# pedroand6/Voxel-Raytracer

Measured on AMD Instinct MI355X. Metric: Mrays/s at 1920×1080 primary rays; achieved HBM GB/s vs peak, higher is better.
Workload: dtype f32

## Files before the change

voxel-raytracer_amd/__init__.py:

```python
import ctypes as C
import os
import subprocess

import numpy as np

HERE = os.path.dirname(os.path.abspath(__file__))
CSRC = os.path.join(HERE, "csrc")
HIP_LIB = os.environ.get("VRT_HIP_LIB") or os.path.join(HERE, "libvrt_hip.so")
HOST_LIB = os.path.join(HERE, "libvrt_host.so")
TEST_LIB = os.path.join(HERE, "libvrt_hip_test.so")
OPT_RAY_TABLES, OPT_EMPTY_OCTANTS, OPT_DISPLAY_KERNEL, OPT_FULL_OPAQUE, OPT_HEAVY_TILES, OPT_MISS_TILES = 1, 2, 3, 4, 5, 6

MODE_PRIMARY, MODE_PRIMARY_SHADOW, MODE_FULL = 0, 1, 2
MODES = {"primary": MODE_PRIMARY, "primary_shadow": MODE_PRIMARY_SHADOW, "full": MODE_FULL}
ACCUM_JITTER = 1
TONEMAP_CLAMP, TONEMAP_REINHARD = 0, 1
TONEMAPS = {"clamp": TONEMAP_CLAMP, "reinhard": TONEMAP_REINHARD}


class Tonemap(C.Structure):
    _fields_ = [("op", C.c_int32), ("exposure", C.c_float)]


class VrtError(RuntimeError):
# ... 501 lines not shown
    cp = np.ascontiguousarray(cam_pos, np.float32)
    iv = np.ascontiguousarray(inv_view, np.float32)
    out = (C.c_int32 * 12)()
    r = L.vrt_test_lens_select(t.ctypes.data if t.size else None, t.size, (C.c_int32 * 3)(*world_min), (C.c_int32 * 3)(*world_max),
                               float(voxel_scale), _fptr(cp), _fptr(iv), float(aperture), out)
    if r != 0:
        raise VrtError(f"vrt_test_lens_select failed ({r})")
    return dict(box_valid=bool(out[0]), eye_shared=bool(out[1]), first_shared=bool(out[2]), no_medium=bool(out[3]),
                empty=bool(out[4]), lo=tuple(out[5:8]), hi=tuple(out[8:11]), root_shift=int(out[11]))


def miss_mask(texels, inv_proj, inv_view, cam_pos, width, height, voxel_scale=1.0, world_min=(-1023, -1023, -1023),
              world_max=(1024, 1024, 1024)):
    L = test_lib()
    L.vrt_test_miss_mask.argtypes = [C.c_void_p, C.c_size_t, C.POINTER(C.c_int32), C.POINTER(C.c_int32), C.c_float,
                                     C.POINTER(C.c_float), C.POINTER(C.c_float), C.POINTER(C.c_float), C.c_int, C.c_int,
                                     C.c_void_p, C.POINTER(C.c_int32)]
    t = np.ascontiguousarray(texels, np.uint8)
    ip = np.ascontiguousarray(inv_proj, np.float32).reshape(-1)
    iv = np.ascontiguousarray(inv_view, np.float32).reshape(-1)
    cp = np.zeros(4, np.float32)
    cp[:len(cam_pos)] = np.asarray(cam_pos, np.float32).reshape(-1)[:4]
    mask = np.zeros(((height + 7) // 8, (width + 7) // 8), np.uint8)
    stats = (C.c_int32 * 2)()
    r = L.vrt_test_miss_mask(t.ctypes.data if t.size else None, t.size, (C.c_int32 * 3)(*world_min), (C.c_int32 * 3)(*world_max),
                             float(voxel_scale), _fptr(ip), _fptr(iv), _fptr(cp), int(width), int(height), mask.ctypes.data, stats)
    if r < 0:
        raise VrtError(f"vrt_test_miss_mask failed ({r})")
    if r == 0:
        return None
    return mask, int(stats[0]), bool(stats[1])


def test_tile_order(tile_ticks, wave_slots, device=0):
    L = test_lib()
    t = np.ascontiguousarray(tile_ticks, np.uint32).reshape(-1)
    assert t.size % 4 == 0
    n = t.size // 4
    L.vrt_test_tile_order.argtypes = [C.c_int, C.c_void_p, C.c_uint32, C.c_uint32, C.c_void_p, C.c_void_p]
    order = np.zeros(n, np.uint32)
    split = np.zeros(1, np.uint32)
    r = L.vrt_test_tile_order(device, t.ctypes.data, n, wave_slots, order.ctypes.data, split.ctypes.data)
    if r:
        raise VrtError(f"vrt_test_tile_order failed ({r})")
    return order, int(split[0])



def tree_is_opaque(texels):
    L = test_lib()
    L.vrt_test_tree_is_opaque.argtypes = [C.c_void_p, C.c_size_t]
    t = np.ascontiguousarray(texels, np.uint8)
    r = L.vrt_test_tree_is_opaque(t.ctypes.data if t.size else None, t.size)
    if r < 0:
        raise VrtError(f"vrt_test_tree_is_opaque failed ({r})")
    return r == 1


def view_in_range(inv_view):
    m = np.ascontiguousarray(inv_view, np.float32).reshape(16)
    return test_lib().vrt_test_view_in_range(m.ctypes.data) == 1


def wide_find(texels, points, world_min=(-1023, -1023, -1023), world_max=(1024, 1024, 1024)):
    L = test_lib()
    t = np.ascontiguousarray(texels, np.uint8)
# ... 525 lines not shown
```

voxel-raytracer_amd/csrc/vrt_args.h:

```cpp
#pragma once
#include <hip/hip_runtime.h>
#include <stdint.h>

namespace vrt {

struct F3 { float x, y, z; };
struct I3 { int x, y, z; };

constexpr int kMaxViews = 4;
constexpr int kGroupTiles = 4;
constexpr int kSplitParts = 8, kSplitMaxGroups = 64;
struct View {
    float inv_proj[16];
    float inv_view[16];
    float cam_pos[4];
    uint32_t *out_rgba;
    int2 *out_id;
    uint32_t eye0, eye1;
    uint32_t first_w0, first_w1, first_node, first_anode;
    int first_s, first_as, first_valid;
    const float *gen_x, *gen_y;
    float gen_z;
    uint32_t gen_fast;
    const uint8_t *miss;
    uint32_t miss_stamp;
};

struct ViewSet {
    View v[kMaxViews];
};

struct KArgs {
    int n_views;
    float voxel_scale;
    int wmin[3];
    int wmax[3];
    float global_light[4];
    float light_dir[3];
    float light_inv[3], light_push[3], light_dposf[3];
    int light_dpos[3];
    int shade_fast;
    int highlighted[3];
    int tex_dim;
    int width, height;
    int row0, n_rows, tile_rows, row_stride;
    int compact;
    uint32_t tiles_x_magic;
    int row_mode;
    const uint2 *nodes;
    uint32_t n_records;
    uint32_t lds_records;
    const uint2 *cells;
    const uint2 *cells4;
    uint32_t n_roots;
    const uint32_t *root_table;
    uint32_t root0_node;
    int root0_shift;
// ... 15 lines not shown
```

voxel-raytracer_amd/csrc/vrt_common.hip.h:

```cpp
#pragma once

#include "vrt_args.h"

namespace vrt {

#define VRT_DEV __device__ __forceinline__

VRT_DEV float fmin_c(float a, float b) { return b < a ? b : a; }
VRT_DEV float fmax_c(float a, float b) { return a < b ? b : a; }
VRT_DEV float dot3(F3 a, F3 b) { return (a.x * b.x + a.y * b.y) + a.z * b.z; }
VRT_DEV float len3(F3 a) { return __builtin_sqrtf(dot3(a, a)); }
VRT_DEV F3 scale3(F3 a, float s) { return F3{a.x * s, a.y * s, a.z * s}; }
VRT_DEV F3 add3(F3 a, F3 b) { return F3{a.x + b.x, a.y + b.y, a.z + b.z}; }
VRT_DEV F3 sub3(F3 a, F3 b) { return F3{a.x - b.x, a.y - b.y, a.z - b.z}; }
VRT_DEV F3 normalize3(F3 a) { return scale3(a, 1.0f / __builtin_sqrtf(dot3(a, a))); }

VRT_DEV float rcp_inrange(float x) {
    float y = __builtin_amdgcn_rcpf(x);
    y = __builtin_fmaf(__builtin_fmaf(-x, y, 1.0f), y, y);
    const float q = __builtin_fmaf(__builtin_fmaf(-x, y, 1.0f), y, y);
    return __builtin_fmaf(__builtin_fmaf(-x, q, 1.0f), y, q);
}
VRT_DEV float sqrt_inrange(float x) {
    const float s = __builtin_amdgcn_sqrtf(x);
// ... 186 lines not shown
}

VRT_DEV void record_find(const KArgs &a, I3 p, uint32_t &w0, uint32_t &w1) {
    w0 = w1 = 0u;
    if (!in_world(a, p)) return;
    int mn[3] = {a.wmin[0], a.wmin[1], a.wmin[2]}, mx[3] = {a.wmax[0], a.wmax[1], a.wmax[2]};
    const int q[3] = {p.x, p.y, p.z};
    uint32_t rec = 0u;
    for (int i = 0; i < 16; ++i) {
        uint32_t ci = 0u;
#pragma unroll
        for (int k = 0; k < 3; ++k) {
            const int mid = mn[k] + ((mx[k] - mn[k]) >> 1);
            const bool hi = q[k] >= mid;
            if (hi) { ci |= 1u << (2 - k); mn[k] = mid; } else mx[k] = mid;
        }
        const uint2 r = a.nodes[rec];
        const uint32_t bit = 1u << ci;
        if (!(r.x & bit)) return;
        const uint32_t idx = r.y + (uint32_t)__builtin_popcount(r.x & 0xffu & (bit - 1u));
        if (idx >= a.n_records) return;
        if (r.x & (bit << 8)) { const uint2 l = a.nodes[idx]; w0 = l.x; w1 = l.y; return; }
        rec = idx;
    }
}

template <class T, class = void> struct host_light { static constexpr bool value = false; };
template <class T> struct host_light<T, decltype((void)T::kHostLight)> { static constexpr bool value = T::kHostLight; };
template <class T, class = void> struct miss_tiles { static constexpr bool value = false; };
template <class T> struct miss_tiles<T, decltype((void)T::kMissTiles)> { static constexpr bool value = T::kMissTiles; };

VRT_DEV bool miss_forward(F3 d) {
    return (d.x > 0.0f || d.x < -2e-8f) && (d.y > 0.0f || d.y < -2e-8f) && (d.z > 0.0f || d.z < -2e-8f);
}

constexpr uint32_t kSeedPlanes = 5, kSeedValid = 1u << 31;
struct Seed { F3 hp; uint32_t word; float iof; };

template <int MODE, class TRAV, bool JIT = false, bool LENS = false, bool MISS = false, bool HDR = false>
VRT_DEV void trace_pixel(const KArgs &a, const View &vw, const typename TRAV::Ctx &tc_, int px, int py, uint32_t &rgba, int2 &idd, LateOut &lo,
                         uint32_t *seed = nullptr, Seed *seed_regs = nullptr, uint32_t sample = 0u, const LensRay *lens = nullptr,
                         uint32_t miss_byte = 0u, float *fc_out = nullptr) {
    const float kPI = 3.14159265359f;
    const LensRay pr = pixel_ray<JIT, LENS>(a, vw, px, py, sample, lens);
    F3 ray_dir = pr.dir, ray_origin = pr.o;
    uint32_t eye0 = pr.eye0, eye1 = pr.eye1;

    int voxel_id = 0;
    int pixel_dist = a.wmax[0] - a.wmin[0];
    F3 gro = scale3(ray_origin, a.voxel_scale);
    Decoded tvd = decode_leaf(eye0, eye1);
    float start_iof = (tvd.p[0] > 0.0f && tvd.p[0] < 3.0f) ? tvd.p[0] : 1.0f;
    float medium_density = tvd.c[3] * 5.0f;
    float mc[3] = {1.0f, 1.0f, 1.0f};
    if (tvd.c[3] > 0.0f) { mc[0] = tvd.c[0]; mc[1] = tvd.c[1]; mc[2] = tvd.c[2]; }
    float fc[3] = {0.0f, 0.0f, 0.0f};
    const float sky[3] = {0.5f, 0.7f, 1.0f};

    Hit h;
    uint32_t seed_word = 0u;
    float seed_iof = 1.0f;
    const uint32_t eye_b = eye1 & 0xffu;
    const uint32_t iof_byte = (eye_b >= 1u && eye_b <= 254u) ? eye_b : 85u;
    bool hit = false;
    bool miss_tile = false;
    if constexpr (MISS) {
// ... 191 lines not shown
            uint32_t rgba;
            int2 idd;
            const View &vw = vs.v[blockIdx.y];
            LateOut lo;
            if constexpr (MODE == 5) {
                const uint32_t *sp = reinterpret_cast<const uint32_t *>(a.defer_rec) + ((size_t)tile * kSeedPlanes) * 64 + lane;
                Seed seed;
                seed.word = sp[3 * 64];
                seed.hp = F3{0.0f, 0.0f, 0.0f};
                seed.iof = 1.0f;
                if (seed.word & kSeedValid) {
                    seed.hp = F3{__uint_as_float(sp[0]), __uint_as_float(sp[64]), __uint_as_float(sp[2 * 64])};
                    seed.iof = __uint_as_float(sp[4 * 64]);
                }
                if (full::bounce_pixel<TRAV>(a, tc_, px, py, seed, rgba)) {
                    const LateArgs la = late_args();
                    const LateView lv_ = late_view();
                    lv_->out_rgba[(size_t)(la->compact ? j : py) * (size_t)la->width + (size_t)px] = rgba;
                }
            } else {
            if constexpr (MODE == 2)
                full::trace_pixel_full<TRAV>(a, vw, tc_, px, py, rgba, idd, lo);
            else if constexpr (MODE == 4)
                trace_pixel<1, TRAV>(a, vw, tc_, px, py, rgba, idd, lo, reinterpret_cast<uint32_t *>(a.defer_rec) + ((size_t)tile * kSeedPlanes) * 64 + lane);
            else if constexpr (MODE == 6) {
                Seed seed;
                seed.word = 0u;
                trace_pixel<1, TRAV>(a, vw, tc_, px, py, rgba, idd, lo, nullptr, &seed);
                uint32_t both;
                if (full::bounce_pixel<TRAV>(a, tc_, px, py, seed, both)) rgba = both;
            }
            else if constexpr ((MODE == 0 || MODE == 1) && miss_tiles<TRAV>::value) {
                uint32_t miss_byte = vw.miss_stamp;
                if (vw.miss) {
                    miss_byte = vw.miss[8u + (uint32_t)(py >> 3) * (uint32_t)((a.width + 7) >> 3) + (uint32_t)(px >> 3)];
                    if (*reinterpret_cast<const uint32_t *>(vw.miss) == vw.miss_stamp) miss_byte = vw.miss_stamp;
                }
                trace_pixel<MODE, TRAV, false, false, true>(a, vw, tc_, px, py, rgba, idd, lo, nullptr, nullptr, 0u, nullptr, miss_byte);
            }
            else trace_pixel<MODE, TRAV>(a, vw, tc_, px, py, rgba, idd, lo);
            if constexpr (MODE == 0) lo = LateOut{vw.out_rgba, vw.out_id, a.width, a.compact};
            size_t o = (size_t)(lo.compact ? j : py) * (size_t)lo.width + (size_t)px;
            if (lo.out_rgba) lo.out_rgba[o] = rgba;
            if (lo.out_id) lo.out_id[o] = idd;
            }
        }
        if constexpr (SCHED & 2) {
#ifndef VRT_EXP_STATS
            if (part_wave) { if (lane == 0) atomicMax(&a.tile_cost[tile], (uint32_t)(((__builtin_readcyclecounter() - t_begin) * 21ull) >> 4)); }
            else if (lane == 0) a.tile_cost[tile] = (uint32_t)(__builtin_readcyclecounter() - t_begin);
#endif
        }
    }
}

}
```

voxel-raytracer_amd/csrc/vrt_dispatch.cpp:

```cpp
#include "vrt_internal.h"

#include <algorithm>
#include <cmath>
#include <cstdio>
#include <new>

using namespace vrt_internal;
#include "vrt_launch.h"

namespace vrt_internal {

SchedState *sched_state(vrt_ctx *c, hipStream_t s, int width, int n_rows, int row0, int row_stride, int tile_rows, int mode,
                        uint32_t n_tiles, uint32_t n_groups) {
    uint64_t &tick = c->sched_tick;
    ++tick;
    for (SchedState &st : c->sched)
        if (st.stream == s && st.width == width && st.n_rows == n_rows && st.row0 == row0 && st.row_stride == row_stride &&
            st.tile_rows == tile_rows && st.mode == mode && st.n_tiles == n_tiles && st.n_groups == n_groups) {
            st.last_use = tick;
            return &st;
        }
    SchedState *slot = nullptr;
    if (c->sched.size() < kSchedMaxStates) {
        c->sched.emplace_back();
// ... 84 lines not shown
    if (hipMemcpy(t->d_tab, tab.data(), tab.size() * sizeof(float), hipMemcpyHostToDevice) != hipSuccess) return nullptr;
    t->fit_ok = miss_table_fit(tab.data(), z, W, H, t->fit);
    t->ok = true;
    return t;
}

bool occupancy(vrt_ctx *c) {
    vrt_ctx::Occupancy &o = c->occ;
    const bool same = o.built && o.tree_gen == c->tree_gen && std::memcmp(o.wmin, c->params.world_min, sizeof o.wmin) == 0 &&
                      std::memcmp(o.wmax, c->params.world_max, sizeof o.wmax) == 0;
    if (same) return o.ok;
    o.built = true; o.ok = false;
    o.tree_gen = c->tree_gen;
    std::memcpy(o.wmin, c->params.world_min, sizeof o.wmin);
    std::memcpy(o.wmax, c->params.world_max, sizeof o.wmax);
    for (int k = 0; k < 3; ++k)
        if (o.wmin[k] < -vrt::miss::kMaxWorld || o.wmax[k] > vrt::miss::kMaxWorld) return false;
    std::vector<int> boxes;
    if (!vrt::occupancy_boxes(c->host_records, o.wmin, o.wmax, (size_t)vrt::miss::kMaxBoxes, boxes)) return false;
    const size_t bytes = boxes.size() * sizeof(int);
    if (hipDeviceSynchronize() != hipSuccess) return false;
    if (bytes > o.capacity) {
        (void)hipFree(o.d_boxes);
        o.d_boxes = nullptr; o.capacity = 0;
        if (hipMalloc((void **)&o.d_boxes, bytes) != hipSuccess) { (void)hipGetLastError(); return false; }
        o.capacity = bytes;
    }
    if (bytes && hipMemcpy(o.d_boxes, boxes.data(), bytes, hipMemcpyHostToDevice) != hipSuccess) { (void)hipGetLastError(); return false; }
    o.n_boxes = boxes.size() / 6;
    o.ok = true;
    return true;
}

const uint8_t *miss_mask(vrt_ctx *c, const vrt::View &w, const vrt_ctx::RayTable &t, float voxel_scale, hipStream_t s, uint32_t &stamp) {
    vrt_ctx::Occupancy &o = c->occ;
    if (o.seen_gen != c->tree_gen || std::memcmp(o.seen_wmin, c->params.world_min, sizeof o.seen_wmin) != 0 ||
        std::memcmp(o.seen_wmax, c->params.world_max, sizeof o.seen_wmax) != 0) {
        o.seen_gen = c->tree_gen;
        std::memcpy(o.seen_wmin, c->params.world_min, sizeof o.seen_wmin);
        std::memcpy(o.seen_wmax, c->params.world_max, sizeof o.seen_wmax);
        o.stable = 0;
    }
    const uint64_t need = std::max<uint64_t>(vrt::miss::kStableMin, c->host_records.size() / vrt::miss::kStablePerRecords);
    if (o.stable < need) { ++o.stable; return nullptr; }
    const float gro[3] = {w.cam_pos[0] * voxel_scale, w.cam_pos[1] * voxel_scale, w.cam_pos[2] * voxel_scale};
    if (!vrt::miss::eye_in_world(gro, c->params.world_min, c->params.world_max)) return nullptr;
    const int W = t.width, H = t.height;
    vrt_ctx::MissMask *hit = nullptr, *lru = nullptr;
    for (auto &m : c->miss_masks) {
        if (m.width == W && m.height == H && m.tree_gen == c->tree_gen && std::memcmp(m.wmin, c->params.world_min, sizeof m.wmin) == 0 &&
            std::memcmp(m.wmax, c->params.world_max, sizeof m.wmax) == 0 && std::memcmp(m.inv_proj, w.inv_proj, sizeof m.inv_proj) == 0 &&
            std::memcmp(m.inv_view, w.inv_view, sizeof m.inv_view) == 0 && std::memcmp(m.gro, gro, sizeof m.gro) == 0)
            hit = &m;
        if (!lru || m.last_use < lru->last_use) lru = &m;
    }
    if (hit && !hit->pending) {
        hit->last_use = ++c->miss_tick;
        if (!hit->ok) return nullptr;
        if (hit->stream != s) {
            if (hipStreamWaitEvent(s, hit->built, 0) != hipSuccess) { (void)hipGetLastError(); return nullptr; }
            hit->shared = true;
        }
        stamp = hit->stamp;
        return reinterpret_cast<const uint8_t *>(hit->d_mask);
    }
    if (!hit) {
        vrt_ctx::MissMask *m;
        if (c->miss_masks.size() < 8) {
            c->miss_masks.emplace_back();
            m = &c->miss_masks.back();
        } else {
            m = lru;
        }
        std::memcpy(m->inv_proj, w.inv_proj, sizeof m->inv_proj);
        std::memcpy(m->inv_view, w.inv_view, sizeof m->inv_view);
        std::memcpy(m->gro, gro, sizeof m->gro);
        m->width = W; m->height = H; m->tree_gen = c->tree_gen;
        std::memcpy(m->wmin, c->params.world_min, sizeof m->wmin);
        std::memcpy(m->wmax, c->params.world_max, sizeof m->wmax);
        m->ok = false;
        m->pending = true;
        m->last_use = ++c->miss_tick;
        return nullptr;
    }
    vrt_ctx::MissMask *m = hit;
    m->pending = false;
    m->last_use = ++c->miss_tick;
    vrt::miss::ViewParams vp;
    if (!t.fit_ok || !miss_view_params(w.inv_view, gro, t.fit, vp)) return nullptr;
    if (!m->built && hipEventCreateWithFlags(&m->built, hipEventDisableTiming) != hipSuccess) { m->built = nullptr; (void)hipGetLastError(); return nullptr; }
    if (!occupancy(c)) return nullptr;
    if (m->d_mask && (m->shared || m->stream != s) && hipDeviceSynchronize() != hipSuccess) return nullptr;
    const size_t bytes = 8 + (size_t)vp.tiles_x * (size_t)vp.tiles_y;
    if (bytes > m->capacity) {
        if (m->d_mask && hipDeviceSynchronize() != hipSuccess) return nullptr;
        uint32_t *fresh = nullptr;
        if (hipMalloc((void **)&fresh, bytes) != hipSuccess) { (void)hipGetLastError(); return nullptr; }
        (void)hipFree(m->d_mask);
        m->d_mask = fresh;
        m->capacity = bytes;
        m->stamp = 0;
    }
    if (m->stamp == 255u) m->stamp = 0u;
    m->stamp = (uint8_t)(m->stamp + 1u);
    if (m->stamp == 1u && hipMemsetAsync(m->d_mask, 0, m->capacity, s) != hipSuccess) { (void)hipGetLastError(); return nullptr; }
    if (vrt::launch::miss_mask(vp, c->occ.d_boxes, (uint32_t)c->occ.n_boxes, m->d_mask, m->stamp, s) != hipSuccess ||
        hipEventRecord(m->built, s) != hipSuccess) {
        (void)hipGetLastError();
        return nullptr;
    }
    m->stream = s;
    m->shared = false;
    m->ok = true;
    stamp = m->stamp;
    return reinterpret_cast<const uint8_t *>(m->d_mask);
}

int enqueue(vrt_ctx *c, int width, int height, int row0, int n_rows, int tile_rows, int row_stride, int compact,
            int mode, void *d_rgba, void *d_id, hipStream_t s, const vrt_view *views, int n_views, const AccumStep *acc) {
    if (!c->have_scene) return vrt_fail(c, VRT_E_STATE, "vrt_dispatch: no octree uploaded (call vrt_upload_octree first)");
    if (c->batch.open) return vrt_fail(c, VRT_E_STATE, "vrt_dispatch: a patch batch is open (call vrt_patch_end first)");
    if (!views && !c->have_camera) return vrt_fail(c, VRT_E_STATE, "vrt_dispatch: no camera set (call vrt_set_camera first)");
    if (n_views < 1 || n_views > vrt::kMaxViews) return vrt_fail(c, VRT_E_INVALID, "vrt_dispatch_views: 1 to 4 views per launch");
    if (mode != VRT_MODE_PRIMARY && mode != VRT_MODE_PRIMARY_SHADOW && mode != VRT_MODE_FULL)
        return vrt_fail(c, VRT_E_INVALID, "unknown mode");
    if (n_rows <= 0) return VRT_OK;
    {
        const int ra = ensure_analysis(c);
        if (ra) return ra;
    }
    Variant v = *find_variant(c->variant);
    if (v.trav >= 3 && !c->wide_ok) { v.trav = 2; v.wpe = 1; }
    if (v.trav == 2 && c->unit_internal) v.trav = 1;
    if (mode == VRT_MODE_FULL) {
        if (v.trav >= 3) v.wpe = 5;
    } else if (!acc && mode == VRT_MODE_PRIMARY_SHADOW && c->variant == 20 && v.trav == 3) {
        v.wpe = 7;
    }
    vrt::KArgs a;
    vrt::ViewSet vs;
    std::memset(&vs, 0, sizeof vs);
    a.n_views = n_views;
    int eyes[vrt::kMaxViews][3];
    const vrt_ctx::RayTable *tables[vrt::kMaxViews] = {};
    for (int i = 0; i < n_views; ++i) {
        vrt::View &w = vs.v[i];
        std::memcpy(w.inv_proj, views ? views[i].inv_projection : c->inv_proj, sizeof w.inv_proj);
        std::memcpy(w.inv_view, views ? views[i].inv_view : c->inv_view, sizeof w.inv_view);
        std::memcpy(w.cam_pos, views ? views[i].camera_pos : c->cam_pos, sizeof w.cam_pos);
        w.out_rgba = (uint32_t *)(views ? views[i].d_rgba8 : d_rgba);
        w.out_id = (int2 *)(views ? views[i].d_id_dist : d_id);
        int eye[3];
        for (int k = 0; k < 3; ++k) {
            const float g = floorf(w.cam_pos[k] * c->params.voxel_scale);
            eye[k] = g != g ? 0 : (g >= 2147483648.0f ? 2147483647 : (g < -2147483648.0f ? (-2147483647 - 1) : (int)g));
        }
        for (int k = 0; k < 3; ++k) eyes[i][k] = eye[k];
        vrt::eye_lookup(c->host_records, c->params.world_min, c->params.world_max, eye, w.eye0, w.eye1);
        vrt::FirstFind ff;
        w.first_valid = (c->wide_ok && vrt::first_find(c->wide, c->params.world_min, c->params.world_max, eye, vrt::v3::kAnchorShift, ff)) ? 1 : 0;
        if (w.first_valid) {
            w.first_w0 = ff.w0; w.first_w1 = ff.w1; w.first_node = ff.node; w.first_anode = ff.anode;
            w.first_s = ff.s; w.first_as = ff.as;
        }
        w.gen_x = w.gen_y = nullptr; w.gen_z = 0.0f; w.gen_fast = 0u;
        w.miss = nullptr;
        w.miss_stamp = 0u;
        tables[i] = nullptr;
        if (view_matrix_in_range(w.inv_view)) {
            if (const vrt_ctx::RayTable *t = ray_table(c, w.inv_proj, width, height)) {
                w.gen_x = t->d_tab; w.gen_y = t->d_tab + width; w.gen_z = t->z; w.gen_fast = 1u;
                tables[i] = t;
            }
        }
    }
    const bool lens = acc && acc->aperture > 0.0f;
    vrt::LensSel lsel;
    if (lens) {
        vrt::lens_select(c->host_records, c->wide_ok ? &c->wide : nullptr, c->params.world_min, c->params.world_max,
                         c->params.voxel_scale, vs.v[0].cam_pos, vs.v[0].inv_view, acc->aperture, lsel);
        if (!lsel.first_shared) vs.v[0].first_valid = 0;
    }
    if (v.trav == 4 && mode != VRT_MODE_FULL) {
        bool eye_in_medium = false;
        for (int i = 0; i < n_views; ++i) {
            const uint32_t b = vs.v[i].eye1 & 0xffu;
            eye_in_medium = eye_in_medium || (b >= 1u && b <= 254u && b != 85u);
        }
        if (lens) eye_in_medium = !lsel.no_medium;
        if (eye_in_medium) { v.trav = 3; v.wpe = 6; }
    }
    if (c->miss_tiles_on && !acc && v.trav == 4 && v.wpe == 7 && mode != VRT_MODE_FULL)
        for (int i = 0; i < n_views; ++i)
            if (tables[i]) vs.v[i].miss = miss_mask(c, vs.v[i], *tables[i], c->params.voxel_scale, s, vs.v[i].miss_stamp);
    a.voxel_scale = c->params.voxel_scale;
    for (int i = 0; i < 3; ++i) {
        a.wmin[i] = c->params.world_min[i];
        a.wmax[i] = c->params.world_max[i];
        a.light_dir[i] = c->params.light_dir[i];
        a.highlighted[i] = c->params.highlighted[i];
        const float d = a.light_dir[i];
        a.light_inv[i] = (fabsf(d) < 1e-8f) ? 1e20f : 1.0f / d;
        a.light_push[i] = (d > 0.0f ? 1.0f : (d < 0.0f ? -1.0f : 0.0f)) * 0.001f;
        a.light_dpos[i] = d > 0.0f ? 1 : 0;
        a.light_dposf[i] = d > 0.0f ? 1.0f : 0.0f;
    }
    for (int i = 0; i < 4; ++i) a.global_light[i] = c->params.global_light[i];
    a.shade_fast = 1;
    for (int i = 0; i < 3; ++i)
        if (!(fabsf(a.global_light[i]) <= 1073741824.0f) || !(fabsf(a.light_dir[i]) <= 1073741824.0f)) a.shade_fast = 0;
    a.tex_dim = (int)c->info.tex_dim;
    a.width = width;
    a.height = height;
    a.row0 = row0;
    a.n_rows = n_rows;
    a.tile_rows = tile_rows;
    a.row_stride = row_stride;
    a.compact = compact;
    a.nodes = c->d_nodes;
    a.n_records = c->info.n_records;
    a.lds_records = 0u;
    a.cells = c->d_cells;
    a.cells4 = c->d_cells ? c->d_cells + c->cells_capacity : nullptr;
    a.n_roots = c->wide_ok ? (uint32_t)c->wide.roots.size() : 0u;
    for (int k = 0; k < 3; ++k) a.root0_min[k] = a.n_roots ? c->wide.roots[0].origin[k] : 0;
    a.root_table = c->d_roots;
    a.root0_node = a.n_roots ? c->wide.roots[0].node : 0u;
// ... 422 lines not shown
```

voxel-raytracer_amd/csrc/vrt_internal.h:

```cpp
#pragma once
#include "../../include/vrt.h"

#include <hip/hip_runtime.h>

#include <cstring>
#include <string>
#include <vector>

#include "vrt_args.h"
#include "vrt_layout.h"
#include "vrt_miss.h"

struct Variant {
    int id;
    int trav;
    int wpe;
    int block() const { return trav >= 3 ? 64 : 256; }
};

inline constexpr Variant kVariants[] = {
    {0, 4, 7},
    {1, 1, 1},
    {4, 2, 1},
    {20, 3, 6},
// ... 78 lines not shown
    struct RayTable {
        float inv_proj[16]{};
        int width = 0, height = 0;
        bool ok = false;
        float z = 0.0f;
        float *d_tab = nullptr;
        bool fit_ok = false;
        vrt::miss::TableFit fit{};
        size_t capacity = 0;
        uint64_t last_use = 0;
    };
    std::vector<RayTable> ray_tables;
    uint64_t ray_tick = 0;
    bool miss_tiles_on = true;
    struct Occupancy {
        bool built = false, ok = false;
        uint64_t tree_gen = 0;
        int wmin[3] = {0, 0, 0}, wmax[3] = {0, 0, 0};
        uint64_t seen_gen = ~0ull;
        int seen_wmin[3] = {0, 0, 0}, seen_wmax[3] = {0, 0, 0};
        uint64_t stable = 0;
        int *d_boxes = nullptr;
        size_t capacity = 0, n_boxes = 0;
    };
    Occupancy occ;
    struct MissMask {
        float inv_proj[16]{}, inv_view[16]{}, gro[3]{};
        int width = 0, height = 0;
        uint64_t tree_gen = 0;
        int wmin[3] = {0, 0, 0}, wmax[3] = {0, 0, 0};
        bool pending = false;
        bool ok = false;
        uint32_t *d_mask = nullptr;
        size_t capacity = 0;
        uint8_t stamp = 0;
        bool shared = false;
        hipStream_t stream = nullptr;
        hipEvent_t built = nullptr;
        uint64_t last_use = 0;
    };
    std::vector<MissMask> miss_masks;
    uint64_t miss_tick = 0;
    bool two_pass_on = true;
    bool heavy_split_on = true;
    int two_pass_form = 6;
    bool scene_opaque = false;
    bool scene_opaque_valid = false;
    struct SeedBuffer { hipStream_t stream = nullptr; uint32_t *d = nullptr; size_t tiles = 0; uint64_t last_use = 0; };
    std::vector<SeedBuffer> seeds;
    uint64_t seed_tick = 0;
    bool tight_root_on = true;
    bool root0_only_on = true;
    bool ray_tables_on = true;
    uint64_t tree_gen = 0;
    struct Accum {
        bool begun = false;
        int width = 0, height = 0;
        uint32_t first = 0;
        uint32_t total = 0;
        bool pass1 = false;
        int mode = VRT_MODE_FULL;
        uint32_t flags = 0;
        bool frame = false;
        float inv_proj[16]{}, inv_view[16]{}, cam_pos[4]{};
        float lens[2] = {0.0f, 1.0f};
        vrt_params params{};
// ... 75 lines not shown
```

voxel-raytracer_amd/csrc/vrt_launch.h:

```cpp
#pragma once
#include "vrt_internal.h"
#include "vrt_query.h"
#include "vrt_accum.h"
#include "vrt_rays.h"

namespace vrt {
namespace launch {

hipError_t trace_primary(const Variant &v, const KArgs &a, const ViewSet &vs, int grid, hipStream_t s, hipEvent_t ev0, hipEvent_t ev1);
hipError_t trace_shadow(const Variant &v, const KArgs &a, const ViewSet &vs, int grid, hipStream_t s, hipEvent_t ev0, hipEvent_t ev1);
hipError_t trace_full(const Variant &v, const KArgs &a, const ViewSet &vs, int grid, hipStream_t s, hipEvent_t ev0, hipEvent_t ev1);
hipError_t trace_full_opaque(const KArgs &a, const ViewSet &vs, int grid, int wpe, hipStream_t s, hipEvent_t ev0, hipEvent_t ev1);
hipError_t trace_full_two_pass(const KArgs &a, const ViewSet &vs, int grid, hipStream_t s, hipEvent_t ev0, hipEvent_t ev1);
hipError_t trace_full_pass1(const KArgs &a, const ViewSet &vs, int grid, hipStream_t s);
inline hipError_t trace(int mode, const Variant &v, const KArgs &a, const ViewSet &vs, int grid, hipStream_t s, hipEvent_t ev0, hipEvent_t ev1) {
    return mode == VRT_MODE_FULL ? trace_full(v, a, vs, grid, s, ev0, ev1)
                                 : (mode == VRT_MODE_PRIMARY ? trace_primary(v, a, vs, grid, s, ev0, ev1) : trace_shadow(v, a, vs, grid, s, ev0, ev1));
}

hipError_t tile_order(const uint32_t *d_cost, uint32_t n_groups, uint32_t *d_order, uint32_t wave_slots, bool raise_lds, size_t lds_ceiling, hipStream_t s);
hipError_t miss_mask(const miss::ViewParams &v, const int *d_boxes, uint32_t n, uint32_t *d_mask, uint8_t stamp, hipStream_t s);
hipError_t kernarg_probe(const KArgs &a, const ViewSet &vs, uint32_t *d_bad, hipStream_t s);

struct Denoise {
    const void *rgba, *id;
    void *out;
    int width, height;
    const uint32_t *group_order;
    uint32_t *tile_cost;
    int rows_path = 0;
};
void denoise_tiling(int width, int height, int &tiles_x, int &n_tiles);
hipError_t denoise(const Denoise &d, bool whole_groups, hipStream_t s);

hipError_t cast_rays(const KArgs &a, const query::RayArgs &q, hipStream_t s);
hipError_t find_voxels(const KArgs &a, const query::PointArgs &q, hipStream_t s);

hipError_t accum_primary(int mode, accum::Source src, const Variant &v, const KArgs &a, const ViewSet &vs, const accum::AdaptArgs &q,
                         bool adaptive, const accum::Lens &l, int grid, hipStream_t s);
hipError_t accum_opaque(accum::Source src, const KArgs &a, const ViewSet &vs, const accum::AdaptArgs &q, bool adaptive, const accum::Lens &l,
                        int grid, hipStream_t s);
hipError_t accum_full(accum::Source src, const Variant &v, const KArgs &a, const ViewSet &vs, const accum::AdaptArgs &q, bool adaptive,
                      const accum::Lens &l, int grid, hipStream_t s);
hipError_t accum_bounce(const KArgs &a, const ViewSet &vs, const accum::AdaptArgs &q, bool adaptive, int grid, hipStream_t s);
hipError_t accum_repeat(const accum::Repeat &q, hipStream_t s);
hipError_t accum_repeat(const accum::RepeatAdapt &q, hipStream_t s);
hipError_t accum_resolve(const accum::Resolve &q, hipStream_t s);
hipError_t adaptive_resolve(const accum::Resolve &q, hipStream_t s);
hipError_t adaptive_tiles(const accum::Tiles &t, hipStream_t s);
hipError_t adaptive_counts(const accum::Counts &c, hipStream_t s);

hipError_t accum_primary_hdr(int mode, accum::Source src, const Variant &v, const KArgs &a, const ViewSet &vs, const accum::HdrArgs &q,
                             bool adaptive, const accum::Lens &l, int grid, hipStream_t s);
hipError_t accum_opaque_hdr(accum::Source src, const KArgs &a, const ViewSet &vs, const accum::HdrArgs &q, bool adaptive, const accum::Lens &l,
// ... 16 lines not shown
```

voxel-raytracer_amd/csrc/vrt_launch_misc.hip:

```cpp
#include <hip/hip_runtime.h>

#include "vrt_launch.h"
#include "vrt_sched.hip.h"
#include "vrt_denoise.hip.h"

namespace vrt {
namespace launch {

hipError_t tile_order(const uint32_t *d_cost, uint32_t n_groups, uint32_t *d_order, uint32_t wave_slots, bool raise_lds, size_t lds_ceiling, hipStream_t s) {
    const size_t lds = (size_t)n_groups * sizeof(uint32_t);
    if (raise_lds) {
        const hipError_t e = hipFuncSetAttribute(reinterpret_cast<const void *>(&tile_order_kernel), hipFuncAttributeMaxDynamicSharedMemorySize, (int)lds_ceiling);
        if (e != hipSuccess) return e;
    }
    hipLaunchKernelGGL(tile_order_kernel, dim3(1), dim3(1024), lds, s, (const uint4 *)d_cost, n_groups, d_order, wave_slots);
    return hipGetLastError();
}

constexpr uint32_t kMissLanes = 8;
__global__ __launch_bounds__(256) void miss_mask_kernel(const miss::ViewParams v, const miss::Box *boxes, uint32_t n, uint32_t *hdr,
                                                        uint32_t stamp) {
    uint8_t *mask = reinterpret_cast<uint8_t *>(hdr + 2);
    const uint32_t g = blockIdx.x * blockDim.x + threadIdx.x;
    const uint32_t i = g / kMissLanes, c = g % kMissLanes;
    if (i >= n) return;
    miss::Extent e = miss::project_corner(v, boxes[i], (int)c);
    for (int d = 1; d < (int)kMissLanes; d <<= 1) {
        miss::Extent o;
        o.lo_x = __shfl_xor(e.lo_x, d, kMissLanes); o.hi_x = __shfl_xor(e.hi_x, d, kMissLanes);
        o.lo_y = __shfl_xor(e.lo_y, d, kMissLanes); o.hi_y = __shfl_xor(e.hi_y, d, kMissLanes);
        o.behind = __shfl_xor(e.behind, d, kMissLanes); o.near = __shfl_xor(e.near, d, kMissLanes);
        e = miss::merge_extent(e, o);
    }
    int t[4];
    const int r = miss::extent_tiles(v, e, t);
    if (r == 2 && c == 0) hdr[0] = stamp;
    if (r == 1) {
        const uint32_t w = (uint32_t)(t[2] - t[0] + 1), cnt = w * (uint32_t)(t[3] - t[1] + 1);
        for (uint32_t k = c; k < cnt; k += kMissLanes) mask[(uint32_t)(t[1] + (int)(k / w)) * (uint32_t)v.tiles_x + (uint32_t)t[0] + k % w] = (uint8_t)stamp;
    }
}

hipError_t miss_mask(const miss::ViewParams &v, const int *d_boxes, uint32_t n, uint32_t *d_mask, uint8_t stamp, hipStream_t s) {
    const uint32_t blocks = n ? (uint32_t)(((uint64_t)n * kMissLanes + 255u) / 256u) : 1u;
    hipLaunchKernelGGL(miss_mask_kernel, dim3(blocks), dim3(256), 0, s, v, reinterpret_cast<const miss::Box *>(d_boxes), n, d_mask,
                       (uint32_t)stamp);
    return hipGetLastError();
}

hipError_t kernarg_probe(const KArgs &a, const ViewSet &vs, uint32_t *d_bad, hipStream_t s) {
    hipLaunchKernelGGL(kernarg_probe_kernel, dim3(1, kMaxViews), dim3(64), 0, s, a, vs, d_bad);
    return hipGetLastError();
}

void denoise_tiling(int width, int height, int &tiles_x, int &n_tiles) {
    tiles_x = (width + denoise::kTW - 1) / denoise::kTW;
    n_tiles = tiles_x * ((height + 15) / 16);
}

hipError_t denoise(const Denoise &d, bool whole_groups, hipStream_t s) {
    using namespace vrt::denoise;
    Args a;
    a.rgba = (const uint32_t *)d.rgba;
    a.id = (const int2 *)d.id;
    a.out = (uint32_t *)d.out;
    a.width = d.width;
    a.height = d.height;
    denoise_tiling(d.width, d.height, a.tiles_x, a.n_tiles);
    a.group_order = d.group_order;
    a.tile_cost = d.tile_cost;
    a.rows_path = d.rows_path;
    if (!whole_groups) {
        const dim3 grid((unsigned)a.tiles_x, (unsigned)(a.n_tiles / a.tiles_x));
        hipLaunchKernelGGL((denoise_px_kernel<2, 16>), grid, dim3(kTW / 2, 16), 0, s, a);
    } else {
        const long groups = ((long)a.n_tiles + kGroupTiles - 1) / kGroupTiles;
        hipLaunchKernelGGL((denoise_px_kernel<2, 16, true>), dim3((unsigned)(groups * kGroupTiles)), dim3(kTW / 2, 16), 0, s, a);
    }
    return hipGetLastError();
// ... 5 lines not shown
```

voxel-raytracer_amd/csrc/vrt_miss.h:

```cpp
#pragma once
#include <stdint.h>

#if defined(__HIPCC__) || defined(__HIP__)
#define VRT_MISS_HD __host__ __device__ inline
#else
#define VRT_MISS_HD inline
#endif

namespace vrt {
namespace miss {

constexpr int kTile = 8;
constexpr double kDilate = 1.0;
constexpr double kMinDepth = 0.25;
constexpr int kMaxBoxes = 1 << 21;
constexpr double kMaxEye = 65536.0;
constexpr int kStableMin = 64;
constexpr int kStablePerRecords = 512;
constexpr int kMaxWorld = 2048;

struct Box { int mn[3], mx[3]; };

VRT_MISS_HD bool eye_in_world(const float gro[3], const int wmin[3], const int wmax[3]) {
    for (int k = 0; k < 3; ++k)
        if (!((double)gro[k] >= (double)wmin[k] && (double)gro[k] < (double)wmax[k])) return false;
    return true;
}

struct ViewParams {
    double m[9];
    double eye[3];
    double gx0, gdx;
    double gy0, gdy;
    double gz;
    double margin_px;
    int width, height, tiles_x, tiles_y;
};

struct TableFit {
    double gx0, gdx, gy0, gdy, gz;
    double dev_px;
    double gmax2;
    int width, height;
};

struct Extent {
    double lo_x, hi_x, lo_y, hi_y;
    int behind;
    int near;
};
VRT_MISS_HD Extent empty_extent() { return Extent{1e300, -1e300, 1e300, -1e300, 0, 0}; }
VRT_MISS_HD Extent project_corner(const ViewParams &v, const Box &b, int c) {
    const double p[3] = {(double)((c & 1) ? b.mx[0] : b.mn[0]) + ((c & 1) ? kDilate : -kDilate) - v.eye[0],
                         (double)((c & 2) ? b.mx[1] : b.mn[1]) + ((c & 2) ? kDilate : -kDilate) - v.eye[1],
                         (double)((c & 4) ? b.mx[2] : b.mn[2]) + ((c & 4) ? kDilate : -kDilate) - v.eye[2]};
    const double qx = v.m[0] * p[0] + v.m[1] * p[1] + v.m[2] * p[2];
    const double qy = v.m[3] * p[0] + v.m[4] * p[1] + v.m[5] * p[2];
    const double qz = v.m[6] * p[0] + v.m[7] * p[1] + v.m[8] * p[2];
    const double depth = qz / v.gz;
    Extent e = empty_extent();
    if (depth < 0.0) { e.behind = 1; return e; }
    if (!(depth >= kMinDepth)) { e.near = 1; return e; }
    const double gx = qx / depth, gy = qy / depth;
    e.lo_x = e.hi_x = gx;
    e.lo_y = e.hi_y = gy;
    return e;
}
VRT_MISS_HD Extent merge_extent(Extent a, Extent b) {
    a.lo_x = b.lo_x < a.lo_x ? b.lo_x : a.lo_x; a.hi_x = b.hi_x > a.hi_x ? b.hi_x : a.hi_x;
    a.lo_y = b.lo_y < a.lo_y ? b.lo_y : a.lo_y; a.hi_y = b.hi_y > a.hi_y ? b.hi_y : a.hi_y;
    a.behind += b.behind; a.near += b.near;
    return a;
}
// ... 2 lines not shown
    if (e.behind == 8) return 0;
    if (e.behind || e.near) return 2;
    double px0 = (e.lo_x - v.gx0) / v.gdx, px1 = (e.hi_x - v.gx0) / v.gdx;
    double py0 = (e.lo_y - v.gy0) / v.gdy, py1 = (e.hi_y - v.gy0) / v.gdy;
    if (px0 > px1) { const double s = px0; px0 = px1; px1 = s; }
    if (py0 > py1) { const double s = py0; py0 = py1; py1 = s; }
    px0 -= v.margin_px; px1 += v.margin_px; py0 -= v.margin_px; py1 += v.margin_px;
    if (!(px0 == px0) || !(px1 == px1) || !(py0 == py0) || !(py1 == py1)) return 2;
    if (px1 < 0.0 || py1 < 0.0 || px0 > (double)(v.width - 1) || py0 > (double)(v.height - 1)) return 0;
    const double x0 = px0 < 0.0 ? 0.0 : px0, y0 = py0 < 0.0 ? 0.0 : py0;
    const double x1 = px1 > (double)(v.width - 1) ? (double)(v.width - 1) : px1;
    const double y1 = py1 > (double)(v.height - 1) ? (double)(v.height - 1) : py1;
    t[0] = (int)x0 / kTile; t[1] = (int)y0 / kTile;
    t[2] = (int)x1 / kTile; t[3] = (int)y1 / kTile;
    return 1;
}

VRT_MISS_HD int box_tiles(const ViewParams &v, const Box &b, int t[4]) {
    Extent e = empty_extent();
    for (int c = 0; c < 8; ++c) e = merge_extent(e, project_corner(v, b, c));
    return extent_tiles(v, e, t);
}

VRT_MISS_HD bool mark_box(const ViewParams &v, const Box &b, uint8_t *mask, uint8_t stamp) {
    int t[4];
    const int r = box_tiles(v, b, t);
    if (r == 2) return true;
    if (r == 1)
        for (int ty = t[1]; ty <= t[3]; ++ty)
            for (int tx = t[0]; tx <= t[2]; ++tx) mask[ty * v.tiles_x + tx] = stamp;
    return false;
}

}
}
```

voxel-raytracer_amd/csrc/vrt_raygen.cpp:

```cpp
#include <cmath>
#include <cstring>
#include <vector>

#include "vrt_miss.h"

namespace vrt_internal {

bool build_ray_table(const float *m, int W, int H, std::vector<float> &tab, float &z_out) {
    static const int kZeros[10] = {4, 8, 12, 1, 9, 13, 2, 6, 3, 7};
    for (int k : kZeros)
        if (!(m[k] == 0.0f)) return false;
    const auto row = [&](int r, float u, float v) {
        return (m[0 * 4 + r] * u + m[1 * 4 + r] * v) + (m[2 * 4 + r] * -1.0f + m[3 * 4 + r] * 1.0f);
    };
    const auto same = [](float a, float b) { return std::memcmp(&a, &b, sizeof a) == 0; };
    const float w = row(3, 1.0f, 1.0f), z = row(2, 1.0f, 1.0f);
    for (int k = 1; k < 4; ++k) {
        const float u = (k & 1) ? -1.0f : 1.0f, v = (k & 2) ? -1.0f : 1.0f;
        if (!same(row(3, u, v), w) || !same(row(2, u, v), z)) return false;
    }
    if (!(w == w) || !(z == z)) return false;
    const bool divide = fabsf(w) > 1e-6f;
    tab.resize((size_t)W + (size_t)H);
    double hi = 0.0;
// ... 12 lines not shown
        if (!same(y, row(1, -1.0f, v))) return false;
        const float q = divide ? y / w : y;
        if (!(fabs((double)q) <= 1.0995e12)) return false;
        tab[(size_t)W + (size_t)py] = q;
    }
    z_out = divide ? z / w : z;
    const double az = fabs((double)z_out);
    return az >= 9.0949e-13 && az <= 1.0995e12;
}

bool view_matrix_in_range(const float *m) {
    double a[3][3], f2 = 0.0;
    for (int c = 0; c < 3; ++c)
        for (int r = 0; r < 3; ++r) { a[r][c] = (double)m[c * 4 + r]; f2 += a[r][c] * a[r][c]; }
    if (!(f2 >= 9.0949e-13 && f2 <= 1.0995e12)) return false;
    const double det = a[0][0] * (a[1][1] * a[2][2] - a[1][2] * a[2][1]) - a[0][1] * (a[1][0] * a[2][2] - a[1][2] * a[2][0]) +
                       a[0][2] * (a[1][0] * a[2][1] - a[1][1] * a[2][0]);
    return det * det >= 2.3842e-7 * f2 * f2 * f2;
}

bool miss_table_fit(const float *tab, float z, int W, int H, vrt::miss::TableFit &f) {
    if (W < 1 || H < 1) return false;
    const float *tx = tab, *ty = tab + W;
    f.gx0 = tx[0]; f.gdx = W > 1 ? ((double)tx[W - 1] - (double)tx[0]) / (double)(W - 1) : 1.0;
    f.gy0 = ty[0]; f.gdy = H > 1 ? ((double)ty[H - 1] - (double)ty[0]) / (double)(H - 1) : 1.0;
    f.gz = z;
    if (!(std::fabs(f.gdx) > 0.0) || !(std::fabs(f.gdy) > 0.0) || !(std::fabs(f.gz) > 0.0)) return false;
    double dev = 0.0;
    for (int px = 0; px < W; ++px) dev = std::fmax(dev, std::fabs(((double)tx[px] - (f.gx0 + px * f.gdx)) / f.gdx));
    for (int py = 0; py < H; ++py) dev = std::fmax(dev, std::fabs(((double)ty[py] - (f.gy0 + py * f.gdy)) / f.gdy));
    const double xm = std::fmax(std::fabs((double)tx[0]), std::fabs((double)tx[W - 1]));
    const double ym = std::fmax(std::fabs((double)ty[0]), std::fabs((double)ty[H - 1]));
    f.dev_px = dev;
    f.gmax2 = xm * xm + ym * ym + f.gz * f.gz;
    f.width = W; f.height = H;
    return dev == dev && f.gmax2 == f.gmax2;
}

bool miss_view_params(const float *inv_view, const float gro[3], const vrt::miss::TableFit &f, vrt::miss::ViewParams &v) {
    double a[3][3], f2 = 0.0;
    for (int c = 0; c < 3; ++c)
        for (int r = 0; r < 3; ++r) { a[r][c] = (double)inv_view[c * 4 + r]; f2 += a[r][c] * a[r][c]; }
    const double det = a[0][0] * (a[1][1] * a[2][2] - a[1][2] * a[2][1]) - a[0][1] * (a[1][0] * a[2][2] - a[1][2] * a[2][0]) +
                       a[0][2] * (a[1][0] * a[2][1] - a[1][1] * a[2][0]);
    if (!(std::fabs(det) > 0.0) || !std::isfinite(det)) return false;
    double g2 = 0.0;
    for (int r = 0; r < 3; ++r)
        for (int c = 0; c < 3; ++c) {
            const int r0 = (c + 1) % 3, r1 = (c + 2) % 3, c0 = (r + 1) % 3, c1 = (r + 2) % 3;
            v.m[r * 3 + c] = (a[r0][c0] * a[r1][c1] - a[r0][c1] * a[r1][c0]) / det;
            g2 += v.m[r * 3 + c] * v.m[r * 3 + c];
        }
    for (int k = 0; k < 3; ++k) {
        if (!(std::fabs((double)gro[k]) <= vrt::miss::kMaxEye)) return false;
        v.eye[k] = (double)gro[k];
    }
    v.gx0 = f.gx0; v.gdx = f.gdx; v.gy0 = f.gy0; v.gdy = f.gdy; v.gz = f.gz;
    const double eps = 1e-5 * std::sqrt(f2 * g2);
    const double err = eps * f.gmax2 / std::fabs(f.gz) / std::fmin(std::fabs(f.gdx), std::fabs(f.gdy));
    v.margin_px = 1.5 + f.dev_px + err;
    if (!(v.margin_px <= 16.0)) return false;
    v.width = f.width; v.height = f.height;
    v.tiles_x = (f.width + vrt::miss::kTile - 1) / vrt::miss::kTile;
    v.tiles_y = (f.height + vrt::miss::kTile - 1) / vrt::miss::kTile;
    return true;
}

}
```

Before: 55200.

## Skip traversal for wavefronts whose tiles are all certified miss with forward rays

Adds a per-tile 'forward' mask, computed by a new kernel from the ray generation tables and view rotation, that certifies every ray in an 8x8 tile has all direction components safely away from zero. When a whole wave's tiles are both marked as misses and forward, the pixel writes the sky color and the miss id directly instead of calling trace_pixel. It adds an extra small kernel launch, a host-side monotonicity check and an extra byte load per pixel. Correctness depends on the conservative bounds matching what the full tracer would compute.

```diff
diff --git a/voxel-raytracer_amd/__init__.py b/voxel-raytracer_amd/__init__.py
--- a/voxel-raytracer_amd/__init__.py
+++ b/voxel-raytracer_amd/__init__.py
@@ -557,6 +557,31 @@
     return mask, int(stats[0]), bool(stats[1])
 
 
+def miss_forward(inv_proj, inv_view, cam_pos, width, height, voxel_scale=1.0, world_min=(-1023, -1023, -1023),
+                 world_max=(1024, 1024, 1024), eps_scale=1.0, tables=None):
+    L = test_lib()
+    L.vrt_test_miss_forward.argtypes = [C.POINTER(C.c_int32), C.POINTER(C.c_int32), C.c_float, C.POINTER(C.c_float), C.POINTER(C.c_float),
+                                        C.POINTER(C.c_float), C.c_int, C.c_int, C.c_double, C.c_void_p, C.c_void_p, C.POINTER(C.c_double),
+                                        C.c_void_p]
+    ip = np.ascontiguousarray(inv_proj, np.float32).reshape(-1)
+    iv = np.ascontiguousarray(inv_view, np.float32).reshape(-1)
+    cp = np.zeros(4, np.float32)
+    cp[:len(cam_pos)] = np.asarray(cam_pos, np.float32).reshape(-1)[:4]
+    fwd = np.zeros(((height + 7) // 8, (width + 7) // 8), np.uint8)
+    tab = np.zeros(width + height + 1, np.float32)
+    eps = C.c_double(0.0)
+    tin = None if tables is None else np.ascontiguousarray(tables, np.float32).reshape(-1)
+    assert tin is None or tin.size == width + height
+    r = L.vrt_test_miss_forward((C.c_int32 * 3)(*world_min), (C.c_int32 * 3)(*world_max), float(voxel_scale), _fptr(ip), _fptr(iv), _fptr(cp),
+                                int(width), int(height), float(eps_scale), fwd.ctypes.data, tab.ctypes.data, C.byref(eps),
+                                None if tin is None else tin.ctypes.data)
+    if r < 0:
+        raise VrtError(f"vrt_test_miss_forward failed ({r})")
+    if r == 0:
+        return None
+    return fwd, tab[:width], tab[width:width + height], float(tab[width + height]), float(eps.value)
+
+
 def test_tile_order(tile_ticks, wave_slots, device=0):
     L = test_lib()
     t = np.ascontiguousarray(tile_ticks, np.uint32).reshape(-1)
diff --git a/voxel-raytracer_amd/csrc/vrt_args.h b/voxel-raytracer_amd/csrc/vrt_args.h
--- a/voxel-raytracer_amd/csrc/vrt_args.h
+++ b/voxel-raytracer_amd/csrc/vrt_args.h
@@ -23,6 +23,7 @@
     float gen_z;
     uint32_t gen_fast;
     const uint8_t *miss;
+    const uint8_t *miss_fwd;
     uint32_t miss_stamp;
 };
 
diff --git a/voxel-raytracer_amd/csrc/vrt_common.hip.h b/voxel-raytracer_amd/csrc/vrt_common.hip.h
--- a/voxel-raytracer_amd/csrc/vrt_common.hip.h
+++ b/voxel-raytracer_amd/csrc/vrt_common.hip.h
@@ -242,6 +242,14 @@
 
 VRT_DEV bool miss_forward(F3 d) {
     return (d.x > 0.0f || d.x < -2e-8f) && (d.y > 0.0f || d.y < -2e-8f) && (d.z > 0.0f || d.z < -2e-8f);
+}
+
+VRT_DEV uint32_t miss_rgba(float gl0, float gl1, float gl2) {
+    const float gl[3] = {gl0, gl1, gl2}, sky[3] = {0.5f, 0.7f, 1.0f};
+    float fc[3] = {0.0f, 0.0f, 0.0f};
+#pragma unroll
+    for (int k = 0; k < 3; ++k) fc[k] = fc[k] + gl[k] * sky[k] * gl[k] * 1.0f;
+    return unorm8(fc[0]) | (unorm8(fc[1]) << 8) | (unorm8(fc[2]) << 16) | (255u << 24);
 }
 
 constexpr uint32_t kSeedPlanes = 5, kSeedValid = 1u << 31;
@@ -499,10 +507,27 @@
             }
             else if constexpr ((MODE == 0 || MODE == 1) && miss_tiles<TRAV>::value) {
                 uint32_t miss_byte = vw.miss_stamp;
+                bool all_miss = false;
                 if (vw.miss) {
-                    miss_byte = vw.miss[8u + (uint32_t)(py >> 3) * (uint32_t)((a.width + 7) >> 3) + (uint32_t)(px >> 3)];
+                    const uint32_t at = (uint32_t)(py >> 3) * (uint32_t)((a.width + 7) >> 3) + (uint32_t)(px >> 3);
+                    miss_byte = vw.miss[8u + at];
                     if (*reinterpret_cast<const uint32_t *>(vw.miss) == vw.miss_stamp) miss_byte = vw.miss_stamp;
+                    else if (vw.miss_fwd) {
+                        uint32_t fwd_byte = vw.miss_fwd[at];
+                        asm volatile("" : "+v"(miss_byte), "+v"(fwd_byte));
+                        all_miss = __builtin_amdgcn_ballot_w64((miss_byte == vw.miss_stamp) | (fwd_byte != vw.miss_stamp)) == 0ull;
+                    }
                 }
+                if (all_miss) {
+                    if constexpr (MODE == 1) {
+                        const LateArgs la = late_args();
+                        lo = late_out(la, late_view());
+                        rgba = miss_rgba(la->global_light[0], la->global_light[1], la->global_light[2]);
+                    } else {
+                        rgba = miss_rgba(a.global_light[0], a.global_light[1], a.global_light[2]);
+                    }
+                    idd = make_int2(0, a.wmax[0] - a.wmin[0]);
+                } else
                 trace_pixel<MODE, TRAV, false, false, true>(a, vw, tc_, px, py, rgba, idd, lo, nullptr, nullptr, 0u, nullptr, miss_byte);
             }
             else trace_pixel<MODE, TRAV>(a, vw, tc_, px, py, rgba, idd, lo);
diff --git a/voxel-raytracer_amd/csrc/vrt_dispatch.cpp b/voxel-raytracer_amd/csrc/vrt_dispatch.cpp
--- a/voxel-raytracer_amd/csrc/vrt_dispatch.cpp
+++ b/voxel-raytracer_amd/csrc/vrt_dispatch.cpp
@@ -140,7 +140,9 @@
     return true;
 }
 
-const uint8_t *miss_mask(vrt_ctx *c, const vrt::View &w, const vrt_ctx::RayTable &t, float voxel_scale, hipStream_t s, uint32_t &stamp) {
+const uint8_t *miss_mask(vrt_ctx *c, const vrt::View &w, const vrt_ctx::RayTable &t, float voxel_scale, hipStream_t s, uint32_t &stamp,
+                         const uint8_t *&fwd) {
+    fwd = nullptr;
     vrt_ctx::Occupancy &o = c->occ;
     if (o.seen_gen != c->tree_gen || std::memcmp(o.seen_wmin, c->params.world_min, sizeof o.seen_wmin) != 0 ||
         std::memcmp(o.seen_wmax, c->params.world_max, sizeof o.seen_wmax) != 0) {
@@ -170,6 +172,7 @@
             hit->shared = true;
         }
         stamp = hit->stamp;
+        if (hit->fwd_off) fwd = reinterpret_cast<const uint8_t *>(hit->d_mask) + hit->fwd_off;
         return reinterpret_cast<const uint8_t *>(hit->d_mask);
     }
     if (!hit) {
@@ -199,7 +202,8 @@
     if (!m->built && hipEventCreateWithFlags(&m->built, hipEventDisableTiming) != hipSuccess) { m->built = nullptr; (void)hipGetLastError(); return nullptr; }
     if (!occupancy(c)) return nullptr;
     if (m->d_mask && (m->shared || m->stream != s) && hipDeviceSynchronize() != hipSuccess) return nullptr;
-    const size_t bytes = 8 + (size_t)vp.tiles_x * (size_t)vp.tiles_y;
+    const size_t tiles = (size_t)vp.tiles_x * (size_t)vp.tiles_y, fwd_off = 8 + (tiles + 7) / 8 * 8;
+    const size_t bytes = fwd_off + tiles;
     if (bytes > m->capacity) {
         if (m->d_mask && hipDeviceSynchronize() != hipSuccess) return nullptr;
         uint32_t *fresh = nullptr;
@@ -212,7 +216,9 @@
     if (m->stamp == 255u) m->stamp = 0u;
     m->stamp = (uint8_t)(m->stamp + 1u);
     if (m->stamp == 1u && hipMemsetAsync(m->d_mask, 0, m->capacity, s) != hipSuccess) { (void)hipGetLastError(); return nullptr; }
-    if (vrt::launch::miss_mask(vp, c->occ.d_boxes, (uint32_t)c->occ.n_boxes, m->d_mask, m->stamp, s) != hipSuccess ||
+    m->fwd_off = t.fit.monotone ? fwd_off : 0;
+    uint8_t *d_fwd = m->fwd_off ? reinterpret_cast<uint8_t *>(m->d_mask) + m->fwd_off : nullptr;
+    if (vrt::launch::miss_mask(vp, c->occ.d_boxes, (uint32_t)c->occ.n_boxes, m->d_mask, m->stamp, t.d_tab, t.d_tab + W, d_fwd, s) != hipSuccess ||
         hipEventRecord(m->built, s) != hipSuccess) {
         (void)hipGetLastError();
         return nullptr;
@@ -221,6 +227,7 @@
     m->shared = false;
     m->ok = true;
     stamp = m->stamp;
+    fwd = d_fwd;
     return reinterpret_cast<const uint8_t *>(m->d_mask);
 }
 
@@ -272,7 +279,7 @@
             w.first_s = ff.s; w.first_as = ff.as;
         }
         w.gen_x = w.gen_y = nullptr; w.gen_z = 0.0f; w.gen_fast = 0u;
-        w.miss = nullptr;
+        w.miss = w.miss_fwd = nullptr;
         w.miss_stamp = 0u;
         tables[i] = nullptr;
         if (view_matrix_in_range(w.inv_view)) {
@@ -300,7 +307,7 @@
     }
     if (c->miss_tiles_on && !acc && v.trav == 4 && v.wpe == 7 && mode != VRT_MODE_FULL)
         for (int i = 0; i < n_views; ++i)
-            if (tables[i]) vs.v[i].miss = miss_mask(c, vs.v[i], *tables[i], c->params.voxel_scale, s, vs.v[i].miss_stamp);
+            if (tables[i]) vs.v[i].miss = miss_mask(c, vs.v[i], *tables[i], c->params.voxel_scale, s, vs.v[i].miss_stamp, vs.v[i].miss_fwd);
     a.voxel_scale = c->params.voxel_scale;
     for (int i = 0; i < 3; ++i) {
         a.wmin[i] = c->params.world_min[i];
diff --git a/voxel-raytracer_amd/csrc/vrt_internal.h b/voxel-raytracer_amd/csrc/vrt_internal.h
--- a/voxel-raytracer_amd/csrc/vrt_internal.h
+++ b/voxel-raytracer_amd/csrc/vrt_internal.h
@@ -134,6 +134,7 @@
         bool pending = false;
         bool ok = false;
         uint32_t *d_mask = nullptr;
+        size_t fwd_off = 0;
         size_t capacity = 0;
         uint8_t stamp = 0;
         bool shared = false;
diff --git a/voxel-raytracer_amd/csrc/vrt_launch.h b/voxel-raytracer_amd/csrc/vrt_launch.h
--- a/voxel-raytracer_amd/csrc/vrt_launch.h
+++ b/voxel-raytracer_amd/csrc/vrt_launch.h
@@ -19,7 +19,8 @@
 }
 
 hipError_t tile_order(const uint32_t *d_cost, uint32_t n_groups, uint32_t *d_order, uint32_t wave_slots, bool raise_lds, size_t lds_ceiling, hipStream_t s);
-hipError_t miss_mask(const miss::ViewParams &v, const int *d_boxes, uint32_t n, uint32_t *d_mask, uint8_t stamp, hipStream_t s);
+hipError_t miss_mask(const miss::ViewParams &v, const int *d_boxes, uint32_t n, uint32_t *d_mask, uint8_t stamp, const float *d_gen_x,
+                     const float *d_gen_y, uint8_t *d_fwd, hipStream_t s);
 hipError_t kernarg_probe(const KArgs &a, const ViewSet &vs, uint32_t *d_bad, hipStream_t s);
 
 struct Denoise {
diff --git a/voxel-raytracer_amd/csrc/vrt_launch_misc.hip b/voxel-raytracer_amd/csrc/vrt_launch_misc.hip
--- a/voxel-raytracer_amd/csrc/vrt_launch_misc.hip
+++ b/voxel-raytracer_amd/csrc/vrt_launch_misc.hip
@@ -41,10 +41,24 @@
     }
 }
 
-hipError_t miss_mask(const miss::ViewParams &v, const int *d_boxes, uint32_t n, uint32_t *d_mask, uint8_t stamp, hipStream_t s) {
+__global__ __launch_bounds__(256) void miss_forward_kernel(const miss::ViewParams v, const float *gen_x, const float *gen_y, uint8_t *fwd,
+                                                           uint32_t stamp) {
+    const uint32_t t = blockIdx.x * blockDim.x + threadIdx.x;
+    if (t >= (uint32_t)v.tiles_x * (uint32_t)v.tiles_y) return;
+    int x0, x1, y0, y1;
+    miss::tile_span(v, (int)(t % (uint32_t)v.tiles_x), (int)(t / (uint32_t)v.tiles_x), x0, x1, y0, y1);
+    if (miss::tile_forward(v, (double)gen_x[x0], (double)gen_x[x1], (double)gen_y[y0], (double)gen_y[y1])) fwd[t] = (uint8_t)stamp;
+}
+
+hipError_t miss_mask(const miss::ViewParams &v, const int *d_boxes, uint32_t n, uint32_t *d_mask, uint8_t stamp, const float *d_gen_x,
+                     const float *d_gen_y, uint8_t *d_fwd, hipStream_t s) {
     const uint32_t blocks = n ? (uint32_t)(((uint64_t)n * kMissLanes + 255u) / 256u) : 1u;
     hipLaunchKernelGGL(miss_mask_kernel, dim3(blocks), dim3(256), 0, s, v, reinterpret_cast<const miss::Box *>(d_boxes), n, d_mask,
                        (uint32_t)stamp);
+    if (d_fwd) {
+        const uint32_t tiles = (uint32_t)v.tiles_x * (uint32_t)v.tiles_y;
+        hipLaunchKernelGGL(miss_forward_kernel, dim3((tiles + 255u) / 256u), dim3(256), 0, s, v, d_gen_x, d_gen_y, d_fwd, (uint32_t)stamp);
+    }
     return hipGetLastError();
 }
 
diff --git a/voxel-raytracer_amd/csrc/vrt_miss.h b/voxel-raytracer_amd/csrc/vrt_miss.h
--- a/voxel-raytracer_amd/csrc/vrt_miss.h
+++ b/voxel-raytracer_amd/csrc/vrt_miss.h
@@ -35,10 +35,15 @@
     double gz;
     double margin_px;
     int width, height, tiles_x, tiles_y;
+    double r[9];
+    double fwd_min;
 };
+
+constexpr double kFwdRel = 1e-5, kFwdAbs = 2e-8;
 
 struct TableFit {
     double gx0, gdx, gy0, gdy, gz;
+    bool monotone;
     double dev_px;
     double gmax2;
     int width, height;
@@ -107,5 +112,27 @@
     return false;
 }
 
+VRT_MISS_HD bool tile_forward(const ViewParams &v, double gx_a, double gx_b, double gy_a, double gy_b) {
+    const double xm = (gx_a < 0.0 ? -gx_a : gx_a) > (gx_b < 0.0 ? -gx_b : gx_b) ? gx_a : gx_b;
+    const double ym = (gy_a < 0.0 ? -gy_a : gy_a) > (gy_b < 0.0 ? -gy_b : gy_b) ? gy_a : gy_b;
+    const double g2 = xm * xm + ym * ym + v.gz * v.gz;
+    const double need2 = v.fwd_min * v.fwd_min * g2;
+    for (int k = 0; k < 3; ++k) {
+        int pos = 0, neg = 0;
+        for (int c = 0; c < 4; ++c) {
+            const double d = v.r[3 * k] * ((c & 1) ? gx_b : gx_a) + v.r[3 * k + 1] * ((c & 2) ? gy_b : gy_a) + v.r[3 * k + 2] * v.gz;
+            if (!(d * d >= need2)) return false;
+            pos += d > 0.0; neg += d < 0.0;
+        }
+        if (pos != 4 && neg != 4) return false;
+    }
+    return true;
+}
+
+VRT_MISS_HD void tile_span(const ViewParams &v, int tx, int ty, int &x0, int &x1, int &y0, int &y1) {
+    x0 = tx * kTile; x1 = x0 + kTile - 1 < v.width - 1 ? x0 + kTile - 1 : v.width - 1;
+    y0 = ty * kTile; y1 = y0 + kTile - 1 < v.height - 1 ? y0 + kTile - 1 : v.height - 1;
+}
+
 }
 }
diff --git a/voxel-raytracer_amd/csrc/vrt_raygen.cpp b/voxel-raytracer_amd/csrc/vrt_raygen.cpp
--- a/voxel-raytracer_amd/csrc/vrt_raygen.cpp
+++ b/voxel-raytracer_amd/csrc/vrt_raygen.cpp
@@ -68,6 +68,10 @@
     const double xm = std::fmax(std::fabs((double)tx[0]), std::fabs((double)tx[W - 1]));
     const double ym = std::fmax(std::fabs((double)ty[0]), std::fabs((double)ty[H - 1]));
     f.dev_px = dev;
+    int up_x = 0, dn_x = 0, up_y = 0, dn_y = 0;
+    for (int px = 1; px < W; ++px) { up_x += tx[px] > tx[px - 1]; dn_x += tx[px] < tx[px - 1]; }
+    for (int py = 1; py < H; ++py) { up_y += ty[py] > ty[py - 1]; dn_y += ty[py] < ty[py - 1]; }
+    f.monotone = !(up_x && dn_x) && !(up_y && dn_y);
     f.gmax2 = xm * xm + ym * ym + f.gz * f.gz;
     f.width = W; f.height = H;
     return dev == dev && f.gmax2 == f.gmax2;
@@ -99,6 +103,9 @@
     v.width = f.width; v.height = f.height;
     v.tiles_x = (f.width + vrt::miss::kTile - 1) / vrt::miss::kTile;
     v.tiles_y = (f.height + vrt::miss::kTile - 1) / vrt::miss::kTile;
+    for (int r = 0; r < 3; ++r)
+        for (int c = 0; c < 3; ++c) v.r[r * 3 + c] = a[r][c];
+    v.fwd_min = (vrt::miss::kFwdRel * std::sqrt(f2 * g2) + vrt::miss::kFwdAbs) * std::sqrt(f2);
     return true;
 }
 
```

Result: no change. 54970 (-0.4%).
